# baoe/AlignGraph

Hardware: AMD Instinct MI355X
Metric: aligned reads/sec through graph build+extend (higher is better)
Workload: dtype u32

## Files before the change

### aligngraph_amd/csrc/agx_walk.cpp

```cpp
#include "agx_host.h"

#include <algorithm>
#include <atomic>
#include <thread>
#include <chrono>
#include <cstdio>
#include <cstdlib>
#include <cstring>
#include <deque>
#include <memory>
#include <memory_resource>
#include <string>
#include <vector>
#include <unordered_map>
#if defined(__x86_64__)
#include <immintrin.h>
#endif

#if defined(AGX_WALK_PROF) && defined(__x86_64__)
#include <x86intrin.h>
static unsigned long long g_prof[12];
#define AGX_PT(i) do { _mm_lfence(); const unsigned long long t_ = __rdtsc(); g_prof[i] += t_ - tp_; tp_ = t_; } while (0)
#define AGX_PT_START _mm_lfence(); unsigned long long tp_ = __rdtsc()
#else
// ... 224 lines not shown
        copies = nullptr;
    }
    bool may_look(agx_u32 v) const { if (!spec) return true; const agx_u32 x = pos_of(v); if (x >= look_lo && x < look_hi) return true; invalid = true; gave_up_at = x; return false; }
    std::vector<agx_edge_ovf> ovf;
    Walker(const UnitView &v, const GraphView &g) : V(v), G(g) {
        if (g.meta_rw) { if (g.meta_rw != g.meta) throw Error{E_ARG, "meta_rw must be the meta array"}; m = g.meta_rw; }
        else {
            const size_t n = (size_t)g.n_ids + 64;
            owned = (agx_u8 *)malloc(n); if (!owned) throw Error{E_ARG, "out of host memory"};
            advise_huge(owned, n); memcpy(owned, g.meta, n); m = owned;
        }
        for (size_t i = 0; i < g.n_ovf; i++) if (g.ovf[i].src != AGX_NONE) ovf.push_back(g.ovf[i]);
        std::sort(ovf.begin(), ovf.end(), [](const agx_edge_ovf &a, const agx_edge_ovf &b) { return a.src != b.src ? a.src < b.src : a.dst < b.dst; });
        ovf.erase(std::unique(ovf.begin(), ovf.end(), [](const agx_edge_ovf &a, const agx_edge_ovf &b) { return a.src == b.src && a.dst == b.dst; }), ovf.end());
    }
    mutable unsigned long long n_fetched = 0;
    mutable std::unordered_map<agx_u32, agx_walknode> extra;
    mutable std::vector<agx_walknode> rows;
    mutable agx_u32 last_v = AGX_NONE, last_at = AGX_NONE;
    agx_u32 rank_of(agx_u32 v) const {
        if (v == last_v) return last_at;
        const unsigned long long w = G.sp_bits[v >> 6], bit = 1ull << (v & 63u);
        last_v = v;
        return last_at = (w & bit) ? G.sp_rank[v >> 6] + (agx_u32)__builtin_popcountll(w & (bit - 1)) : AGX_NONE;
    }
    agx_hop hop_of(agx_u32 v, agx_u32 x) const {
        const agx_u32 r = G.sp_hop ? rank_of(v) : AGX_NONE;
        if (r != AGX_NONE) return G.sp_hop[r];
        if (V.hop) return V.hop[x];
        agx_hop h{0, 0, 0};
        if (!V.segs || V.n_seg0 == 0 || V.cm_count(x) != 1) return h;
        agx_u32 lo = 0, hi = V.n_seg0;
        while (hi - lo > 1) { const agx_u32 mid = lo + (hi - lo) / 2; if (V.segs[mid].pos0 <= x) lo = mid; else hi = mid; }
        const agx_cmseg &g = V.segs[lo];
        const agx_u32 j = x - g.pos0;
        if (x < g.pos0 || j >= g.len || j >= g.hop_len0) return h;
        h.str_off = g.hop_str0 + j; h.len = g.hop_len0 - j; h.end_pos = g.hop_end;
        return h;
    }
    agx_walknode node(agx_u32 v) const {
        const agx_u32 at = rank_of(v);
        if (at != AGX_NONE) {
            if (G.sp_hop) { __builtin_prefetch(G.sp_hop + at); __builtin_prefetch(G.sp_hop + at + 8); }
            __builtin_prefetch(G.sp_node + at + 6);
            return G.sp_node[at];
        }
        const auto it = extra.find(v);
        if (it != extra.end()) return it->second;
        if (!G.fetch) throw Error{E_ARG, "walk graph without a record fetch hook"};
        agx_walknode r; G.fetch(G.fetch_ctx, v, 1, 1, 1, &r); n_fetched++;
        extra.emplace(v, r);
        return r;
    }
    void prefetch_skip_positions(agx_u32 cp, agx_u32 end) const {
        if (!G.fetch || cp + 1000 >= end) return;
        const agx_u32 n = (end - cp - 1) / 1000;
        rows.resize((size_t)n * 2);
        G.fetch(G.fetch_ctx, cp + 999, 1000, n, 2, rows.data());
        for (agx_u32 i = 0; i < n; i++) { extra.emplace(cp + 999 + i * 1000, rows[2 * (size_t)i]); extra.emplace(cp + 1000 + i * 1000, rows[2 * (size_t)i + 1]); }
    }
    agx_u32 pos_of(agx_u32 v) const { return v < G.n_pos ? v : G.side_xpos[v - G.n_pos]; }
    void side_range(agx_u32 x, agx_u32 &lo, agx_u32 &hi) const {
        AGX_WCHK(*this, x, "side_range");
        if (!(m[x] & AGX_WM_SIDE)) { lo = hi = G.n_pos; return; }
        const agx_u32 *b = G.side_xpos, *e = G.side_xpos + (G.n_ids - G.n_pos);
        const agx_u32 *l = std::lower_bound(b, e, x), *h = l;
        while (h < e && *h == x) h++;
        lo = G.n_pos + (agx_u32)(l - b); hi = G.n_pos + (agx_u32)(h - b);
    }
    int live_successors(agx_u32 v, agx_u32 &target) const {
        AGX_WCHK(*this, v, "live_successors");
        if (m[v] & AGX_WM_CONT) { if (spec && v >= G.n_pos && !may_look(v + 1)) return 2; if (visited(v + 1)) return 0; target = v + 1; return 1; }
        int n = 0;
        const agx_walknode rec = node(v);
        const agx_u32 *s = rec.next;
        for (agx_u32 e = 0; e < AGX_MAXE && s[e] != AGX_NONE; e++) { if (!may_look(s[e])) return 2; if (!visited(s[e])) { target = s[e]; if (++n > 1) return n; } }
        if (!ovf.empty()) {
            auto it = std::lower_bound(ovf.begin(), ovf.end(), v, [](const agx_edge_ovf &a, agx_u32 key) { return a.src < key; });
            for (; it != ovf.end() && it->src == v; ++it) {
                bool inl = false; for (agx_u32 e = 0; e < AGX_MAXE; e++) inl |= s[e] == it->dst;
                if (!inl) { if (!may_look(it->dst)) return 2; if (!visited(it->dst)) { target = it->dst; if (++n > 1) return n; } }
            }
        }
        return n;
    }
    void kmer_string(agx_u32 v, std::string &out) const {
        agx_sref r = node(v).sref;
        if (V.slot_row) r.slot = V.slot_row[r.slot];
        const agx_u32 first = r.qlen & 0xFFFFu, len = (r.qlen >> 16) & 0x7FFFu; const bool rev = (r.qlen >> 31) != 0;
        out.clear();
        if (!V.bases) {
            if (!V.codes2) throw Error{E_ARG, "no read bases for the k-mer strings"};
            const agx_u8 *row = V.codes2 + (size_t)r.slot * (V.stride / 4);
            const unsigned long long base = (unsigned long long)r.slot * V.stride;
            for (agx_u32 i = 0; i < len; i++) {
                const agx_u32 j = rev ? first - i : first + i;
                char c = "ACGT"[(row[j >> 2] >> (2u * (j & 3u))) & 3u];
                if (c == 'A' && V.n_other) {
                    const unsigned long long *e = V.other_idx + V.n_other, *at = std::lower_bound(V.other_idx, e, base + j);
                    if (at != e && *at == base + j) c = (char)V.other_byte[at - V.other_idx];
                }
                out.push_back(!rev ? c : c == 'A' ? 'T' : c == 'C' ? 'G' : c == 'G' ? 'C' : c == 'T' ? 'A' : c);
            }
            return;
        }
        const char *p = V.row_off ? V.bases + V.row_off[r.slot] : V.bases + (size_t)(G.row_slot ? G.row_slot[r.slot] : r.slot) * V.stride;
        for (agx_u32 i = 0; i < len; i++) {
            if (!rev) out.push_back(p[first + i]);
            else { const char c = p[first - i]; out.push_back(c == 'A' ? 'T' : c == 'C' ? 'G' : c == 'G' ? 'C' : c == 'T' ? 'A' : c); }
        }
    }
    next_zero_fn next_zero = pick_next_zero();
    agx_u32 next_live(agx_u32 from, agx_u32 n) const { return from < n ? next_zero(m, from, n) : n; }
};

struct WalkState {
    agx_u32 cp = 0;
    agx_u32 seqID = 0, sIDBak = AGX_NONE, sOffBak = AGX_NONE, eIDBak = AGX_NONE, eOffBak = AGX_NONE;
    agx_u32 pos_bak = 0;
    bool same_scan(const WalkState &o) const { return cp == o.cp && sIDBak == o.sIDBak && sOffBak == o.sOffBak && eIDBak == o.eIDBak && eOffBak == o.eOffBak && pos_bak == o.pos_bak; }
};
typedef std::vector<std::pair<agx_u32, agx_u32>> MarkLog;

struct WalkRun {
    Walker &W; Arena *arena;
    WalkState st;
    std::vector<Rec> &written; PreFormat *pre;
    std::vector<PreJob> jobs;
    bool keep = true;
    MarkLog *log = nullptr; agx_u32 log_main = 0, log_side = 0;
    const std::atomic<bool> *cancel = nullptr;
    unsigned long long n_walks = 0, n_hops = 0, n_runs = 0, n_general = 0, run_nodes = 0;
    WalkRun(Walker &w, Arena *a, std::vector<Rec> &out, PreFormat *p) : W(w), arena(a), written(out), pre(p) {}
    void note_marks(agx_u32 a, agx_u32 b) {
        if (a < W.G.n_pos) { if (b >= log_main) log->push_back({a < log_main ? log_main : a, b}); }
        else if (b >= log_side) log->push_back({a < log_side ? log_side : a, b});
    }
    void go(agx_u32 stop) {
        const GraphView &G = W.G; const UnitView &V = W.V;
        agx_u32 &seqID = st.seqID, &sIDBak = st.sIDBak, &sOffBak = st.sOffBak, &eIDBak = st.eIDBak, &eOffBak = st.eOffBak, &pos_bak = st.pos_bak;
        std::string kmer; agx_u32 klen = 0, klast = 0;
        agx_hop hcur{0, 0, 0};
        std::vector<Seg> segs;
        agx_u8 *const m = W.m;
        auto done = [m, this](agx_u32 v) { AGX_WCHK(W, v, "done"); (void)this; return (m[v] & AGX_WM_VISITED) != 0; };
        const mark_fn mark = pick_mark();
        AGX_PT_START;
        const run_end_fn run_end = pick_run_end();
        const agx_u32 n_side = G.n_ids - G.n_pos;
        if (stop > G.n_pos) stop = G.n_pos;
        agx_u32 sc = (agx_u32)(std::lower_bound(G.side_xpos, G.side_xpos + n_side, st.cp) - G.side_xpos);
        agx_u32 side_live = G.n_pos + sc, main_live = st.cp;
        agx_u32 cp = st.cp;
        for (; cp < stop;) {
            if (W.invalid || (cancel && cancel->load(std::memory_order_relaxed))) break;
            while (sc < n_side && G.side_xpos[sc] < cp) sc++;
            agx_u32 sh = sc; while (sh < n_side && G.side_xpos[sh] == cp) sh++;
            const agx_u32 s_lo = G.n_pos + sc, s_hi = G.n_pos + sh;
            for (agx_u32 vi = 0, start = cp; vi <= s_hi - s_lo; vi++, start = s_lo + vi - 1) {
                if (done(start)) continue;
                AGX_PT(8);
                Rec C(arena); C.sID = 0; C.sOff = cp; C.extended = 0;
                segs.clear(); n_walks++;
                agx_u32 cur = start;
                AGX_PT(0);
                agx_u32 cpp = cp; int mode = 1;
                agx_u32 last = cur;
                while ((mode == 1 && !done(cur)) || mode == 0) {
                    if (mode == 0) {
                        AGX_PT(7); const agx_hop h = hcur;
                        segs.push_back(Seg{V.chain_str + h.str_off, h.len}); C.extended = 1; n_hops++;
                        pos_bak = h.end_pos; cpp = h.end_pos;
                        if (!W.may_look(cpp)) { mode = -2; break; }
                        agx_u32 live = 0, item = 0;
                        if (!done(cpp)) { live++; item = cpp; }
                        agx_u32 h_lo, h_hi; W.side_range(cpp, h_lo, h_hi);
                        for (agx_u32 v = h_lo; v < h_hi; v++) if (!done(v)) { live++; item = v; }
                        agx_u32 tgt = 0; int ns = 0;
                        if (live == 1) ns = W.live_successors(item, tgt);
                        if (ns == 1) { cur = tgt; pos_bak = W.pos_of(tgt); cpp = pos_bak; mode = done(cur) ? -2 : 1; }
                        else mode = -2;
                        AGX_PT(1);
                    } else {
                        agx_u8 seen = 0;
                        AGX_WCHK(W, cur, "run start");
                        const agx_u32 j = run_end(m, cur, seen);
                        const agx_u32 xj = j < G.n_ids ? W.pos_of(j) : 0xFFFFFFFFu;
                        if (W.spec && (xj < W.look_lo || xj >= W.look_hi || (j >= G.n_pos && j + 1 < G.n_ids && W.pos_of(j + 1) >= W.look_hi))) { W.invalid = true; W.gave_up_at = xj; mode = -2; break; }
                        AGX_PT(2);
                        AGX_WCHK(W, j, "run end"); if (j + 1 < G.n_ids && (j + 1 < G.n_pos) == (j < G.n_pos)) AGX_WCHK(W, j + 1, "behind the run");
                        segs.push_back(Seg{G.str + cur, (size_t)j - cur + 1}); n_runs++; run_nodes += j - cur + 1; if (!(m[j] & AGX_WM_CONT)) n_general++;
                        if (seen & AGX_WM_CONTIG) C.extended = 1;
                        if (W.copies) W.before_mark(j);
                        mark(m, cur, j);
                        if (log && j >= log_main) note_marks(cur, j);
                        if (j > cur) pos_bak = xj;
                        cur = j; last = j; cpp = xj;
                        AGX_PT(3);
                        agx_u32 tgt = 0;
                        const int ns = (m[cur] & AGX_WM_CONT) ? 0 : W.live_successors(cur, tgt);
                        if (ns == 1) { cur = tgt; pos_bak = W.pos_of(tgt); cpp = pos_bak; }
                        else if ((hcur = W.hop_of(j, xj)).len) mode = 0;
                        else mode = -1;
                        AGX_PT(4);
                    }
                }
                C.eID = 0; C.eOff = mode == 1 ? pos_bak : cpp;
                if (mode == 1 || mode == -1) {
                    { const agx_u32 o = W.node(cur).off0; C.eID0 = o == AGX_NONE ? AGX_NONE : 0; C.eOff0 = o; }
                    klen = (W.node(last).sref.qlen >> 16) & 0x7FFFu; klast = last;
                    C.eOff = C.eOff + klen - 1; C.eOff0 = C.eOff0 + klen - 1;
                } else { C.eID0 = AGX_NONE; C.eOff0 = AGX_NONE; klen = 0; }
                AGX_PT(5);
                if (!contains(sIDBak, sOffBak, eIDBak, eOffBak, C.sID, C.sOff, C.eID, C.eOff)) {
                    { const agx_u32 o = W.node(start).off0; C.sID0 = o == AGX_NONE ? AGX_NONE : 0; C.sOff0 = o; }
                    if (klen > 1) {
                        W.kmer_string(klast, kmer);
                        char *t = (char *)arena->allocate(kmer.size() - 1, 1); memcpy(t, kmer.data() + 1, kmer.size() - 1);
                        segs.push_back(Seg{t, kmer.size() - 1});
                    }
                    C.nuc.segs.reserve(segs.size());
                    for (const Seg &g : segs) C.nuc.add(g.p, g.n);
                    sIDBak = C.sID; sOffBak = C.sOff; eIDBak = C.eID; eOffBak = C.eOff;
                    if (eOffBak - sOffBak > 100000) W.prefetch_skip_positions(cp, eOffBak < G.n_pos ? eOffBak : G.n_pos);
                    if (keep) {
                        PreJob j; const agx_u32 f[10] = {seqID, (agx_u32)C.extended, C.sID, C.sOff, C.eID, C.eOff, C.sID0, C.sOff0, C.eID0, C.eOff0};
                        memcpy(j.f, f, sizeof f); j.segs = C.nuc.segs.data(); j.n_segs = C.nuc.segs.size(); j.total = C.nuc.len;
                        if (pre) pre->add(j); else jobs.push_back(j);
                        written.push_back(std::move(C));
                    }
                    seqID++;
                }
                AGX_PT(6);
            }
            AGX_PT(9);
            if (eOffBak - sOffBak > 100000 && eIDBak == 0 && cp + 1000 < eOffBak) cp += 1000;
            else {
                auto stale = [m](agx_u32 v) { return (m[v] & AGX_WM_VISITED) != 0; };
                if (main_live <= cp || (main_live < G.n_pos && stale(main_live))) main_live = W.next_live(main_live > cp + 1 ? main_live : cp + 1, G.n_pos);
                const agx_u32 m = main_live;
                if (side_live < s_hi || (side_live < G.n_ids && stale(side_live))) side_live = W.next_live(side_live > s_hi ? side_live : s_hi, G.n_ids);
                const agx_u32 sd = side_live;
                const agx_u32 sp = sd < G.n_ids ? G.side_xpos[sd - G.n_pos] : G.n_pos;
                cp = m < sp ? m : sp;
                if (cp >= W.scan_hi) { W.invalid = true; W.gave_up_at = cp; }
            }
            AGX_PT(10);
    }
        st.cp = cp;
    }
};

inline void walk_report(const WalkRun &r) {
#if defined(AGX_WALK_PROF) && defined(__x86_64__)
    if (getenv("AGX_WALK_TIMING")) {
        fprintf(stderr, "[agx walk] Mcycles: start %.1f, hop %.1f, run scan %.1f, mark %.1f, successors %.1f, end %.1f, contain+write %.1f, between %.1f, position scan %.1f (+ %.1f after the last variant, %.1f next position)\n",
                g_prof[0] / 1e6, g_prof[1] / 1e6, g_prof[2] / 1e6, g_prof[3] / 1e6, g_prof[4] / 1e6, g_prof[5] / 1e6, g_prof[6] / 1e6, g_prof[7] / 1e6, g_prof[8] / 1e6, g_prof[9] / 1e6, g_prof[10] / 1e6);
        memset(g_prof, 0, sizeof g_prof);
    }
#endif
    if (getenv("AGX_WALK_TIMING")) fprintf(stderr, "[agx walk] walks %llu, contig hops %llu, runs %llu (%llu nodes), general evaluations %llu\n", r.n_walks, r.n_hops, r.n_runs, r.run_nodes, r.n_general);
}

void walk(Walker &W, OutBuf &pre_out, std::vector<Rec> &written, Arena *arena, Assistant *assistant, WalkPaths *paths) {
    if (W.G.wait_landed) W.G.wait_landed(W.G.land_ctx, W.G.n_pos, W.G.n_ids);
    if (W.G.wait_str) W.G.wait_str(W.G.land_ctx);
    pre_out.reserve((size_t)W.G.n_ids + W.G.n_ids / 32 + 4096);
    PreFormat pre(pre_out, assistant, (size_t)W.G.n_pos / 256 + 65536);
    pre.paths = paths; pre.graph = &W.G;
    WalkRun run(W, arena, written, &pre);
    run.go(W.G.n_pos);
    pre.finish();
    walk_report(run);
}

inline std::atomic<double> &walker_speed() { static std::atomic<double> v{700000.0}; return v; }
inline void clip_marks(const MarkLog &log, agx_u32 main_lo, agx_u32 main_hi, agx_u32 n_pos, agx_u32 side_lo, agx_u32 side_hi, MarkLog &out) {
    out.clear();
    for (const auto &r : log) {
        agx_u32 a = r.first, b = r.second;
        if (b < n_pos) { if (a < main_lo) a = main_lo; if (b >= main_hi) { if (main_hi == 0) continue; b = main_hi - 1; } }
        else { if (a < side_lo) a = side_lo; if (b >= side_hi) { if (side_hi == 0) continue; b = side_hi - 1; } }
        if (a <= b) out.push_back({a, b});
    }
    std::sort(out.begin(), out.end());
    size_t k = 0;
    for (size_t i = 0; i < out.size(); i++) {
        if (k && out[i].first <= out[k - 1].second + 1) { if (out[i].second > out[k - 1].second) out[k - 1].second = out[i].second; }
        else out[k++] = out[i];
    }
    out.resize(k);
}

struct SpecWalker {
    agx_u32 c = 0, c_next = 0, w0 = 0, side_c = 0, side_next = 0, warm_lo = 0, warm_hi = 0xFFFFFFFFu, look_hi = 0, win_lo = 0, win_hi = 0, side_win_hi = 0, copy_hi = 0, side_copy_lo = 0, side_copy_hi = 0;
    Scratch bytes;
    GraphView G; std::unique_ptr<Walker> W; std::unique_ptr<WalkRun> R; std::vector<Rec> recs;
    MarkLog log; size_t n_warm = 0;
    WalkState at_c;
    bool ok = false; std::string error;
    double t_run = 0, t_copy = 0, t_warm = 0, t_done = 0;
};

bool walk_split(Walker &WA, const UnitView &V, const GraphView &G, OutBuf &pre_out, std::vector<Rec> &written, Arena *arena, Arena *const *more_arenas, Assistant *assistant, WalkPaths *paths) {
    const agx_u32 min_ref = getenv("AGX_WALK_SPLIT_MIN") ? (agx_u32)strtoul(getenv("AGX_WALK_SPLIT_MIN"), nullptr, 10) : 4000000u;
    agx_u32 warm = 400000u;
    if (const char *e = getenv("AGX_WALK_SPLIT_WARMUP")) warm = (agx_u32)strtoul(e, nullptr, 10);
    else if (V.segs) {
        agx_u32 reach = 0;
        for (agx_u32 i = 0; i < V.n_seg0; i++) { const agx_cmseg &g = V.segs[i]; if (g.hop_len0 && g.hop_end > g.pos0 && g.hop_end - g.pos0 > reach) reach = g.hop_end - g.pos0; }
        const unsigned long long w = 3ull * reach + 20000ull;
        warm = (agx_u32)(w < 100000ull ? 100000ull : w > 400000ull ? 400000ull : w);
    }
    const agx_u32 n_ref = V.n_ref < G.n_pos ? V.n_ref : G.n_pos;
    if (!assistant || n_ref < min_ref || n_ref < 16 || getenv("AGX_WALK_NO_SPLIT")) return false;
    int K = walkers_for(n_ref);
    if (K > 1 + assistant->helpers()) K = 1 + assistant->helpers();
    const agx_u32 slack = 64;
    if (K > (int)(n_ref / (8 * slack))) K = (int)(n_ref / (8 * slack));
    if (K < 2) return false;
    const agx_u32 lead = n_ref / (unsigned)K > 4 * warm ? 2 * warm : 0;
    std::vector<agx_u32> cuts((size_t)K + 1, n_ref); cuts[0] = 0;
    for (int i = 1; i < K; i++) cuts[(size_t)i] = lead + (agx_u32)((unsigned long long)(n_ref - lead) * (unsigned)i / (unsigned)K);
    const bool streamed = G.wait_landed != nullptr && G.land_ms > 0;
    if (!getenv("AGX_WALK_EVEN_CUTS")) {
        const double v = walker_speed().load(), D = streamed ? G.land_ms : 0.0, copy_ms = 0.15 + 3.2 * ((double)n_ref / K) / 12e6, warm_ms = 2.0 * (double)warm / v, floor_len = std::max(1024.0, (double)n_ref / (16.0 * K));
        std::vector<double> len((size_t)K, (double)n_ref / K), ready((size_t)K, 0.0), at((size_t)K + 1, 0.0);
        for (int round = 0; round < 6; round++) {
            for (int i = 0; i < K; i++) at[(size_t)i + 1] = at[(size_t)i] + len[(size_t)i];
            double sum = ready[0] = D;
            for (int i = 1; i < K; i++) { const double hi = i + 2 >= K ? (double)G.n_pos : std::max(at[(size_t)i + 2], at[(size_t)i + 1] + (double)warm); sum += ready[(size_t)i] = D * std::min(1.0, hi / (double)G.n_pos) + copy_ms + warm_ms; }
            const double T = ((double)n_ref / v + sum) / K;
            double total = 0;
            for (int i = 0; i < K; i++) total += len[(size_t)i] = std::max(v * (T - ready[(size_t)i]), floor_len);
            for (int i = 0; i < K; i++) len[(size_t)i] *= (double)n_ref / total;
        }
        double acc = 0;
        for (int i = 1; i < K; i++) { acc += len[(size_t)i - 1]; const agx_u32 lo = cuts[(size_t)i - 1] + 8 * slack, hi = n_ref - (agx_u32)(K - i) * 8 * slack; const agx_u32 c = (agx_u32)acc; cuts[(size_t)i] = c < lo ? lo : c > hi ? hi : c; }
    }
    auto cut_at = [&](int i) { return i >= K ? n_ref : i <= 0 ? 0u : cuts[(size_t)i]; };
    const agx_u32 n_side = G.n_ids - G.n_pos;
    auto side_of = [&](agx_u32 x) { return G.n_pos + (agx_u32)(std::lower_bound(G.side_xpos, G.side_xpos + n_side, x) - G.side_xpos); };
    const agx_u32 side_ref = side_of(n_ref);
    pre_out.reserve((size_t)G.n_ids + G.n_ids / 32 + 4096);
    const bool timing = getenv("AGX_WALK_TIMING") != nullptr;
    auto clock = [] { return std::chrono::duration<double, std::milli>(std::chrono::steady_clock::now().time_since_epoch()).count(); };

    const double t_enter = clock();
    std::atomic<bool> cancel{false};
    std::atomic<int> copied{0};
    const agx_u8 *const pristine = WA.m;
    std::vector<SpecWalker> B((size_t)K - 1);
    for (int i = 1; i < K; i++) {
        SpecWalker &b = B[(size_t)i - 1];
        b.c = cut_at(i); b.c_next = cut_at(i + 1);
        b.side_c = side_of(b.c); b.side_next = side_of(b.c_next);
        int ahead = i + 2; while (ahead < K && cut_at(ahead) < b.c_next + warm) ahead++;
        const bool open_end = ahead >= K;
        const agx_u32 back = 2 * warm + slack < b.c - cut_at(i - 1) ? 2 * warm + slack : b.c - cut_at(i - 1);
        b.win_lo = b.c - back; b.win_hi = open_end ? n_ref : cut_at(ahead); b.side_win_hi = open_end ? side_ref : side_of(b.win_hi);
        b.copy_hi = open_end ? G.n_pos : b.win_hi; b.side_copy_lo = side_of(b.win_lo); b.side_copy_hi = open_end ? G.n_ids : b.side_win_hi;
        b.warm_lo = b.win_lo ? b.win_lo + slack : 0; b.warm_hi = open_end ? 0xFFFFFFFFu : b.win_hi - slack; b.look_hi = open_end ? n_ref : b.win_hi - slack;
        b.w0 = b.c > warm ? b.c - warm : 0; if (b.w0 < b.warm_lo) b.w0 = b.warm_lo;
        b.bytes.take((size_t)G.n_ids + 64);
        b.G = G; b.G.meta = (const agx_u8 *)b.bytes.p; b.G.meta_rw = (agx_u8 *)b.bytes.p;
        b.W.reset(new Walker(V, b.G));
        b.recs.reserve((size_t)G.n_pos / 2048 + 1024);
        b.R.reset(new WalkRun(*b.W, more_arenas[i - 1], b.recs, nullptr));
    }
    struct Join { Assistant *a; int n; std::atomic<bool> &c; std::vector<bool> joined; void now(int i) { if (!joined[(size_t)i]) { a->wait(i); joined[(size_t)i] = true; } } ~Join() { c.store(true); for (int i = 0; i < n; i++) now(i); } } join{assistant, K - 1, cancel, std::vector<bool>((size_t)K - 1, false)};
    for (int i = 1; i < K; i++) {
        SpecWalker *bp = &B[(size_t)i - 1];
        assistant->run([bp, &cancel, &copied, pristine, &G, n_ref, side_ref] {
            SpecWalker &b = *bp; Walker &W = *b.W; WalkRun &R = *b.R;
            auto clk = [] { return std::chrono::duration<double, std::milli>(std::chrono::steady_clock::now().time_since_epoch()).count(); };
            b.t_run = clk();
            struct Copied { std::atomic<int> &n; bool done = false; void now() { if (!done) { done = true; n.fetch_add(1, std::memory_order_release); } } ~Copied() { now(); } } copied_mark{copied};
            try {
                if (const char *pz = getenv("AGX_WALK_POISON")) { const long v = strtol(pz, nullptr, 0); memset(W.m, v > 1 ? (int)(v & 0xFF) : 0xA5, (size_t)G.n_ids + 64); }
                if (G.wait_landed) G.wait_landed(G.land_ctx, b.copy_hi, b.side_copy_hi);
                memcpy(W.m + b.win_lo, pristine + b.win_lo, (size_t)b.copy_hi - b.win_lo);
                memcpy(W.m + b.side_copy_lo, pristine + b.side_copy_lo, (size_t)b.side_copy_hi - b.side_copy_lo + (b.side_copy_hi == G.n_ids ? 64 : 0));
                if (b.copy_hi < G.n_pos) W.m[b.copy_hi] = AGX_WM_VISITED;
                if (b.side_copy_hi < G.n_ids) W.m[b.side_copy_hi] = AGX_WM_VISITED;
                copied_mark.now(); b.t_copy = clk();
                W.spec = true; W.look_lo = b.warm_lo; W.look_hi = b.warm_hi; W.scan_hi = b.warm_hi;
#ifdef AGX_WALK_CHECK
                W.chk_lo = b.win_lo; W.chk_hi = b.copy_hi; W.chk_slo = b.side_copy_lo; W.chk_shi = b.side_copy_hi;
#endif
                R.cancel = &cancel; R.st.cp = b.w0; R.keep = false; R.log = &b.log; R.log_main = 0; R.log_side = G.n_pos;
                R.go(b.c);
                b.at_c = R.st; b.n_warm = b.log.size(); b.t_warm = clk();
                for (const auto &r : b.log) for (agx_u32 v = r.first; v <= r.second; v++) if (v < G.n_pos ? v >= n_ref : v >= side_ref) W.m[v] &= (agx_u8)~AGX_WM_VISITED;
                R.keep = true; R.st.seqID = 0;
                if (b.c_next < n_ref) { R.log_main = b.c_next; R.log_side = b.side_next; } else R.log = nullptr;
                W.look_lo = b.c; W.look_hi = b.look_hi;
                if (const char *e = getenv("AGX_WALK_SPLIT_LOOK")) { const unsigned long long hi = (unsigned long long)b.c + strtoull(e, nullptr, 10); if (hi < W.look_hi) W.look_hi = (agx_u32)hi; }
                if (!W.invalid && !cancel.load()) R.go(b.c_next);
                b.ok = !W.invalid && !cancel.load() && R.st.cp >= b.c_next; b.t_done = clk();
            } catch (const Error &e) { b.error = e.msg; } catch (const std::exception &e) { b.error = e.what(); }
        }, i - 1);
    }
    WA.copies = &copied; WA.copies_want = K - 1; WA.guard_main = B[0].win_lo; WA.guard_side = B[0].side_copy_lo;
    struct Unguard { Walker &w; ~Unguard() { w.copies = nullptr; } } unguard{WA};
    if (G.wait_landed) G.wait_landed(G.land_ctx, G.n_pos, G.n_ids);

    const double tw0 = clock();
    MarkLog log_a;
    WalkRun A(WA, arena, written, nullptr);
    A.log = &log_a; A.log_main = B[0].c; A.log_side = B[0].side_c;
    A.go(B[0].c);
    A.log = nullptr;
    const size_t a_first = A.jobs.size();
    const double tw1 = clock();
    const MarkLog *truth = &log_a; WalkState at = A.st; int stood = 0; MarkLog ma, mb;
    for (int i = 1; i < K; i++) {
        SpecWalker &b = B[(size_t)i - 1];
        join.now(i - 1);
        bool same = b.ok && b.error.empty() && at.same_scan(b.at_c);
        if (same) {
            MarkLog warm_marks(b.log.begin(), b.log.begin() + (long)b.n_warm);
            clip_marks(*truth, b.c, n_ref, G.n_pos, b.side_c, side_ref, ma); clip_marks(warm_marks, b.c, n_ref, G.n_pos, b.side_c, side_ref, mb);
            same = ma == mb;
        }
        if (timing) {
            if (same) fprintf(stderr, "[agx walk] walker %d of %d, [%u, %u) after a warm-up from %u: its stretch stands (began at %.2f ms, window %.2f ms, warm-up %.2f ms, stretch %.2f ms)\n", i + 1, K, b.c, b.c_next, b.w0, b.t_run - t_enter, b.t_copy - b.t_run, b.t_warm - b.t_copy, b.t_done - b.t_warm);
            else if (!b.error.empty()) fprintf(stderr, "[agx walk] walker %d of %d failed (%s): walked on by the first walker from %u\n", i + 1, K, b.error.c_str(), b.c);
            else if (b.W->invalid) fprintf(stderr, "[agx walk] walker %d of %d gave up (a walk led to position %u, outside [%u, %u)): walked on by the first walker from %u\n", i + 1, K, b.W->gave_up_at, b.W->look_lo, b.W->look_hi, b.c);
            else fprintf(stderr, "[agx walk] walker %d of %d, [%u, %u) after a warm-up from %u: states differ at the meeting point (scan at %u / %u, last record %u..%u / %u..%u, %zu / %zu mark ranges): walked on by the first walker\n",
                         i + 1, K, b.c, b.c_next, b.w0, at.cp, b.at_c.cp, at.sOffBak, at.eOffBak, b.at_c.sOffBak, b.at_c.eOffBak, ma.size(), mb.size());
        }
        if (!same) break;
        const agx_u32 shift = at.seqID;
        for (PreJob &j : b.R->jobs) j.f[0] += shift;
        at = b.R->st; at.seqID = shift + b.R->st.seqID;
        truth = &b.log; stood = i;
    }
    cancel.store(true);
    for (int i = stood; i < K - 1; i++) join.now(i);
    WA.copies = nullptr;
    {
        double pos = 0, ms = 0;
        for (int i = 1; i <= stood; i++) { const SpecWalker &b = B[(size_t)i - 1]; if (b.t_done > b.t_warm) { pos += (double)(b.c_next - b.c); ms += b.t_done - b.t_warm; } }
        if (ms > 0.05 && pos > 1e5) { const double seen = pos / ms, old = walker_speed().load(); walker_speed().store(0.7 * old + 0.3 * std::min(std::max(seen, 1e5), 5e6)); }
    }
    const double tw2 = clock();
    if (!(stood == K - 1 && WA.next_live(n_ref, G.n_pos) >= G.n_pos && WA.next_live(side_ref, G.n_ids) >= G.n_ids)) {
        auto merge = [&WA](const agx_u8 *src, agx_u32 lo, agx_u32 hi) {
            agx_u32 v = lo;
            for (; v < hi && (v & 7u); v++) WA.m[v] |= (agx_u8)(src[v] & AGX_WM_VISITED);
            for (; v + 8 <= hi; v += 8) { uint64_t x, y; memcpy(&x, WA.m + v, 8); memcpy(&y, src + v, 8); x |= y & 0x8080808080808080ull; memcpy(WA.m + v, &x, 8); }
            for (; v < hi; v++) WA.m[v] |= (agx_u8)(src[v] & AGX_WM_VISITED);
        };
        auto merge_of = [&](int i) {
            const SpecWalker &b = B[(size_t)i - 1]; const agx_u8 *src = b.W->m;
            if (i < stood) { merge(src, b.c, b.c_next); merge(src, b.side_c, b.side_next); } else { merge(src, b.c, b.win_hi); merge(src, b.side_c, b.side_win_hi); }
        };
        struct Wait { Assistant *a; int n; ~Wait() { for (int i = 0; i < n; i++) a->wait(i); } } wait{assistant, stood > 1 ? stood - 1 : 0};
        for (int i = 1; i < stood; i++) assistant->run([&merge_of, i] { merge_of(i); }, i - 1);
        if (stood) merge_of(stood);
    }
    for (int i = 1; i <= stood; i++) {
        SpecWalker &b = B[(size_t)i - 1];
        for (Rec &r : b.recs) written.push_back(std::move(r));
        WA.n_fetched += b.W->n_fetched;
        A.n_walks += b.R->n_walks; A.n_hops += b.R->n_hops; A.n_runs += b.R->n_runs; A.n_general += b.R->n_general; A.run_nodes += b.R->run_nodes;
    }
    if (stood) A.st = at;
    const double tw3 = clock();
    A.go(G.n_pos);
    const double tw4 = clock();
    std::vector<PreJob> all;
    all.insert(all.end(), A.jobs.begin(), A.jobs.begin() + (long)a_first);
    for (int i = 1; i <= stood; i++) all.insert(all.end(), B[(size_t)i - 1].R->jobs.begin(), B[(size_t)i - 1].R->jobs.end());
    all.insert(all.end(), A.jobs.begin() + (long)a_first, A.jobs.end());
    if (paths) for (const PreJob &j : all) note_paths(j, G, *paths);
    std::vector<size_t> place(all.size() + 1, 0);
    auto header_len = [](const PreJob &j) { size_t n = 1 + 9 * 2 + 2; for (int i = 0; i < 10; i++) { agx_u32 v = j.f[i]; do { n++; v /= 10u; } while (v); } return n; };
    for (size_t i = 0; i < all.size(); i++) place[i + 1] = place[i] + header_len(all[i]) + all[i].total + (all[i].total + 59) / 60;
    const size_t total = place[all.size()];
    if (G.wait_str) G.wait_str(G.land_ctx);
    pre_out.n = 0; char *base = pre_out.grow(total);
    auto format = [&](size_t lo, size_t hi) {
        for (size_t i = lo; i < hi; i++) {
            const PreJob &j = all[i];
            char *h = base + place[i]; *h++ = '>';
            for (int f = 0; f < 10; f++) { h = put_u32(h, j.f[f]); if (f < 9) { *h++ = ','; *h++ = ' '; } }
            *h++ = ' '; *h++ = '\n';
            LineWriter lw(h); for (size_t g = 0; g < j.n_segs; g++) lw.put(j.segs[g].p, j.segs[g].n); lw.end();
        }
    };
    {
        const int shares = total > (1u << 16) ? K : 1;
        std::vector<size_t> cut((size_t)shares + 1, all.size()); cut[0] = 0;
        for (int t = 1; t < shares; t++) { size_t m = cut[(size_t)t - 1]; while (m < all.size() && place[m] < total / (unsigned)shares * (unsigned)t) m++; cut[(size_t)t] = m; }
        struct Wait { Assistant *a; int n; ~Wait() { for (int i = 0; i < n; i++) a->wait(i); } } wait{assistant, shares - 1};
        for (int t = 0; t + 1 < shares; t++) { const size_t lo = cut[(size_t)t], hi = cut[(size_t)t + 1]; assistant->run([&format, lo, hi] { format(lo, hi); }, t); }
        format(cut[(size_t)shares - 1], all.size());
    }
    if (timing) fprintf(stderr, "[agx walk] first walker began at %.2f ms; %u appended positions behind the reference%s\n", tw0 - t_enter, G.n_pos - n_ref, streamed ? " (streamed download: stretches cut by when their windows land)" : "");
    if (timing && streamed) { fprintf(stderr, "[agx walk] cuts (%.1f ms of download left at the start, %.0f positions per ms):", G.land_ms, walker_speed().load()); for (int i = 1; i < K; i++) fprintf(stderr, " %u", cuts[(size_t)i]); fprintf(stderr, "\n"); }
    if (timing) fprintf(stderr, "[agx walk] %d walkers, %d stretches stood: first stretch %.1f ms, waited %.1f ms for the others, merge %.1f ms, rest %.1f ms, formatting %.1f ms\n", K, stood, tw1 - tw0, tw2 - tw1, tw3 - tw2, tw4 - tw3, clock() - tw4);
    walk_report(A);
    return true;
}

}

namespace {

void join(std::vector<Rec> &c) {
    const int n = (int)c.size();
    for (int cp = 0; cp < n; cp++) if (c[cp].extended == 1)
        for (int q = cp + 1; q < n; q++) {
            if (contains(c[cp].sID, c[cp].sOff, c[cp].eID, c[cp].eOff, c[q].sID, c[q].sOff, c[q].eID, c[q].eOff)) c[q].extended = 2;
            else if (c[cp].eID != c[q].sID || c[cp].eOff < c[q].sOff) break;
        }
    for (int cp = n - 1; cp >= 0; cp--) if (c[cp].extended == 1)
        for (int q = cp - 1; q >= 0; q--) {
            if (contains(c[cp].sID, c[cp].sOff, c[cp].eID, c[cp].eOff, c[q].sID, c[q].sOff, c[q].eID, c[q].eOff)) c[q].extended = 2;
            else if (c[q].eID != c[cp].sID || c[q].eOff < c[cp].sOff) break;
        }
    for (int cp = 0; cp < n; cp++) {
        while (c[cp].extended == 1) {
            int cand = -1, ncand = 0;
            for (int q = cp + 1; q < n; q++) if (c[q].extended != 2) { if (c[cp].eOff >= c[q].sOff) { cand = q; ncand++; } else break; }
            if (ncand != 1) break;
            Rec &d = c[cand]; d.extended = 2;
            const size_t from = (size_t)(int)(c[cp].eOff - d.sOff + 1);
            if (from < d.nuc.len) c[cp].nuc.add_from(d.nuc, from);
            c[cp].eID = d.eID; c[cp].eOff = d.eOff; c[cp].eID0 = d.eID0; c[cp].eOff0 = d.eOff0;
        }
    }
}

inline int overlaps(agx_u32 x1, agx_u32 y1, agx_u32 x2, agx_u32 y2) {
    return (x1 <= x2 && x2 <= y1 && y1 <= y2 && (int)y1 - (int)x2 > 0) || (x2 <= x1 && x1 <= y2 && y2 <= y1 && (int)y2 - (int)x1 > 0) ||
           (x1 <= x2 && x2 <= y2 && y2 <= y1 && (int)y2 - (int)x2 > 0) || (x2 <= x1 && x1 <= y1 && y1 <= y2 && (int)y1 - (int)x1 > 0);
}

void scaffold(const UnitView &V, const GraphView &G, std::vector<Rec> &c, OutBuf &out, Arena *arena, Assistant *assistant) {
    std::vector<Bases> sc; sc.reserve(c.size());
    const agx_u32 n = (agx_u32)c.size();
    std::vector<agx_u32> s_off(n); agx_u32 longest = 0; bool ordered = true;
    for (agx_u32 i = 0; i < n; i++) {
        s_off[i] = c[i].sOff;
        if (i && s_off[i] < s_off[i - 1]) ordered = false;
        if (c[i].eOff < c[i].sOff) longest = 0xFFFFFFFFu; else if (c[i].eOff - c[i].sOff > longest) longest = c[i].eOff - c[i].sOff;
    }
    for (agx_u32 cp = 0; cp < n; cp++) {
        if (!(c[cp].sID != AGX_NONE && c[cp].extended == 1)) continue;
        sc.push_back(std::move(c[cp].nuc)); c[cp].nuc = Bases(arena); c[cp].sID = AGX_NONE;
        bool cont = true;
        while (c[cp].sID0 == c[cp].eID0 && cont) {
            cont = false;
            agx_u32 q = cp + 1;
            if (ordered && longest != 0xFFFFFFFFu && c[cp].sOff0 > longest) {
                const agx_u32 from = (agx_u32)(std::lower_bound(s_off.begin(), s_off.end(), c[cp].sOff0 - longest) - s_off.begin());
                if (from > q) q = from;
            }
            for (; q < n; q++) {
                if (ordered && c[q].sOff > c[cp].eOff0) break;
                if (!(c[cp].eID0 == c[q].sID && c[q].sID == c[q].eID && overlaps(c[cp].sOff0, c[cp].eOff0, c[q].sOff, c[q].eOff) && c[q].extended == 1)) continue;
                if (c[q].sOff > c[cp].eOff) {
                    const agx_u32 gap = c[q].sOff - c[cp].eOff - 1; agx_u32 covered = 0;
                    for (agx_u32 i = 0; i < gap; i++) { const agx_u32 x = c[cp].eOff + i + 1; if ((G.meta[x] & AGX_WM_ANY) || V.has_cm(x)) covered++; }
                    if (gap == 0 || (double)(int)covered / gap >= 0.5) sc.back().add(V.ref + c[cp].eOff + 1, gap);
                    else continue;
                }
                sc.back().add_from(c[q].nuc, 0); c[q].sID = AGX_NONE; cp = q; cont = true;
                break;
            }
        }
    }
    const double t_dec = std::chrono::duration<double, std::milli>(std::chrono::steady_clock::now().time_since_epoch()).count();
    std::vector<size_t> at(sc.size() + 1, 0);
    auto header = [](char *hdr, size_t i) { char *h = hdr; *h++ = '>'; char t[24]; int n = 0; do { t[n++] = (char)('0' + i % 10); i /= 10; } while (i); while (n) *h++ = t[--n]; *h++ = '\n'; return (size_t)(h - hdr); };
    for (size_t i = 0; i < sc.size(); i++) { char hdr[32]; at[i + 1] = at[i] + header(hdr, i) + sc[i].len + (sc[i].len + 59) / 60; }
    const size_t total = at[sc.size()];
    out.n = 0; char *base = out.grow(total);
    auto format = [&](size_t lo, size_t hi) {
        for (size_t i = lo; i < hi; i++) {
            char hdr[32]; const size_t hl = header(hdr, i);
            char *w = base + at[i]; memcpy(w, hdr, hl);
            LineWriter lw(w + hl); lw.put(sc[i]); lw.end();
        }
    };
    const int shares = assistant && total > (1u << 16) ? std::min(8, 1 + assistant->helpers()) : 1;
    if (shares > 1) {
        std::vector<size_t> cut((size_t)shares + 1, sc.size()); cut[0] = 0;
        for (int t = 1; t < shares; t++) { size_t m = cut[(size_t)t - 1]; while (m < sc.size() && at[m] < total / (unsigned)shares * (unsigned)t) m++; cut[(size_t)t] = m; }
        struct Wait { Assistant *a; int n; ~Wait() { for (int i = 0; i < n; i++) a->wait(i); } } wait{assistant, shares - 1};
        for (int t = 0; t + 1 < shares; t++) { const size_t lo = cut[(size_t)t], hi = cut[(size_t)t + 1]; assistant->run([&format, lo, hi] { format(lo, hi); }, t); }
        format(cut[(size_t)shares - 1], sc.size());
    } else format(0, sc.size());
    if (getenv("AGX_WALK_TIMING")) fprintf(stderr, "[agx walk] scaffold: output %.1f ms of it (%zu scaffolds, %zu bytes)\n", std::chrono::duration<double, std::milli>(std::chrono::steady_clock::now().time_since_epoch()).count() - t_dec, sc.size(), total);
}

}

void build_chains(Threads &T) {
    const size_t n = T.cm.size(), n_pos = T.ref.size();
    T.chain_off.assign(1, 0); T.chain_end_pos.clear(); T.chain_str.clear();
    T.chain_str.reserve(n);
    T.hop.assign(n_pos, agx_hop{0, 0, 0});
    std::vector<agx_u8> state(n, 0);
    auto index_of = [&](agx_u32 off, agx_u32 item) -> size_t {
        if (off >= n_pos || T.cm_start[off] + item >= T.cm_start[off + 1]) throw Error{E_ARG, "conti-mer link to a missing entry"};
        return (size_t)T.cm_start[off] + item;
    };
    for (size_t i = 0; i < n; i++) if (T.cm[i].next_off != AGX_NONE) state[index_of(T.cm[i].next_off, T.cm[i].next_item)] = 1;
    std::vector<agx_u32> pending;
    size_t visited = 0;
    T.segs.clear(); T.n_seg0 = 0;
    for (size_t x = 0; x < n_pos; x++) for (size_t h = T.cm_start[x]; h < T.cm_start[x + 1]; h++) {
        if (state[h]) continue;
        pending.clear();
        size_t c = h; agx_u32 pos = (agx_u32)x;
        const size_t seg_first = T.segs.size(), str_base = T.chain_str.size();
        for (agx_u32 i = 0;; i++) {
            if (state[c] == 2) throw Error{E_ARG, "conti-mer chains are not simple lists"};
            state[c] = 2; visited++;
            T.chain_str.push_back(T.cm[c].nuc);
            const ContiMer &m = T.cm[c];
            {
                const agx_u32 rank = (agx_u32)(c - T.cm_start[pos]);
                agx_cmseg *g = T.segs.size() > seg_first ? &T.segs.back() : nullptr;
                const bool joins = g && pos == g->pos0 + g->len && rank == g->rank && m.cid == g->cid && (g->len == 1 || m.coff == g->coff0 + g->len * g->dcoff);
                if (joins) { if (g->len == 1) g->dcoff = m.coff - g->coff0; g->len++; }
                else T.segs.push_back(agx_cmseg{pos, 1u, m.cid, m.coff, 0u, rank, (agx_u32)(str_base + i + 1), i, 0u, 0u});
            }
            if (m.next_off == AGX_NONE) break;
            if (T.cm_start[pos + 1] - T.cm_start[pos] == 1) { T.hop[pos].str_off = (agx_u32)T.chain_str.size(); pending.push_back(pos); }
            c = index_of(m.next_off, m.next_item); pos = m.next_off;
        }
        if (T.chain_str.size() >= 0xFFFFFFFFull) throw Error{E_ARG, "conti-mer chains exceed 2^32 bases"};
        for (agx_u32 p : pending) { T.hop[p].len = (agx_u32)(T.chain_str.size() - T.hop[p].str_off); T.hop[p].end_pos = pos; }
        {   const agx_u32 last = (agx_u32)(T.chain_str.size() - str_base - 1);
            for (size_t g = seg_first; g < T.segs.size(); g++) { T.segs[g].hop_len0 = last - T.segs[g].hop_len0; T.segs[g].hop_end = pos; } }
        T.chain_end_pos.push_back(pos); T.chain_off.push_back(T.chain_str.size());
    }
    if (visited != n) throw Error{E_ARG, "conti-mer cycle"};
    std::stable_sort(T.segs.begin(), T.segs.end(), [](const agx_cmseg &a, const agx_cmseg &b) { return (a.rank != 0) != (b.rank != 0) ? a.rank == 0 : (a.rank == 0 && a.pos0 < b.pos0); });
    agx_u32 e = 0;
    for (agx_cmseg &g : T.segs) { g.elem0 = e; e += g.len; if (g.rank == 0) T.n_seg0++; }
    if (e != n) throw Error{E_ARG, "conti-mer runs do not cover the conti-mers"};
    T.n_cm = n; T.cm_cnt.resize(n_pos);
    for (size_t x = 0; x < n_pos; x++) { const agx_u32 c = T.cm_start[x + 1] - T.cm_start[x]; if (c > 255) throw Error{E_UNSUPPORTED, "more than 255 conti-mers at one position"}; T.cm_cnt[x] = (agx_u8)c; }
}

void walk_join_scaffold(const UnitView &V, const GraphView &G, UnitOutput &out, Assistant *assistant) {
    if (!V.hop && !G.sp_hop && !V.segs) throw Error{E_ARG, "conti-mer chains were not built"};
    const bool timing = getenv("AGX_WALK_TIMING") != nullptr;
    auto now = [] { return std::chrono::duration<double, std::milli>(std::chrono::steady_clock::now().time_since_epoch()).count(); };
    const double ts = now();
    Walker W(V, G);
    std::pmr::monotonic_buffer_resource arena((size_t)8 << 20);
    std::vector<std::unique_ptr<std::pmr::monotonic_buffer_resource>> others;
    Arena *more_arenas[GraphView::MAX_WALKERS - 1];
    for (int i = 0; i < GraphView::MAX_WALKERS - 1; i++) { others.emplace_back(new std::pmr::monotonic_buffer_resource((size_t)1 << 20)); more_arenas[i] = others.back().get(); }
    std::vector<Rec> recs; recs.reserve((size_t)G.n_pos / 1024 + 1024);
    double t0 = now();
    WalkPaths *paths = out.keep_paths ? &out.paths : nullptr;
    if (!walk_split(W, V, G, out.pre_extended, recs, &arena, more_arenas, assistant, paths)) walk(W, out.pre_extended, recs, &arena, assistant, paths);
    double t1 = now();
    join(recs);
    double t2 = now();
    scaffold(V, G, recs, out.extended, &arena, assistant);
    double t3 = now();
    out.n_fetched = W.n_fetched;
    if (timing) fprintf(stderr, "[agx walk] set-up %.2f ms, walk %.2f ms, join %.2f ms, scaffold %.1f ms, %zu records, %u special ids of %u, %llu records fetched\n", t0 - ts, t1 - t0, t2 - t1, t3 - t2, recs.size(), G.n_special, G.n_ids, W.n_fetched);
}

}
```

Before: 1.343 billion.

## Overlap pre-extended output formatting with join and scaffold decisions

Moves the pre-extended FASTA formatting out of walk_split into a PreTail object. Helper threads format the output in dynamically claimed pieces while the unit's thread runs join and the scaffold decisions, and the unit's thread joins in and waits for the helpers before writing the scaffold output. This is meant to take the formatting off the critical path after the last walk stretch. It also replaces the fixed per-walker shares with work-stealing pieces and adds timing instrumentation, at the cost of helper threads being busy when scaffold later wants them.

```diff
diff --git a/aligngraph_amd/csrc/agx_walk.cpp b/aligngraph_amd/csrc/agx_walk.cpp
--- a/aligngraph_amd/csrc/agx_walk.cpp
+++ b/aligngraph_amd/csrc/agx_walk.cpp
@@ -550,7 +550,73 @@
     double t_run = 0, t_copy = 0, t_warm = 0, t_done = 0;
 };
 
-bool walk_split(Walker &WA, const UnitView &V, const GraphView &G, OutBuf &pre_out, std::vector<Rec> &written, Arena *arena, Arena *const *more_arenas, Assistant *assistant, WalkPaths *paths) {
+struct PreTail {
+    std::vector<PreJob> all;
+    std::vector<size_t> place, cut;
+    std::atomic<size_t> next{0};
+    char *base = nullptr; size_t total = 0;
+    const GraphView *G = nullptr; Assistant *assistant = nullptr; int running = 0;
+    bool timing = false; double t_walked = 0, t_started = 0;
+    struct Lap { double begin = 0, bases = 0, end = 0; size_t pieces = 0, bytes = 0; } lap[GraphView::MAX_WALKERS + 1];
+    static double clock() { return std::chrono::duration<double, std::milli>(std::chrono::steady_clock::now().time_since_epoch()).count(); }
+    void format(size_t lo, size_t hi) const {
+        for (size_t i = lo; i < hi; i++) {
+            const PreJob &j = all[i];
+            char *h = base + place[i]; *h++ = '>';
+            for (int f = 0; f < 10; f++) { h = put_u32(h, j.f[f]); if (f < 9) { *h++ = ','; *h++ = ' '; } }
+            *h++ = ' '; *h++ = '\n';
+            LineWriter lw(h); for (size_t g = 0; g < j.n_segs; g++) lw.put(j.segs[g].p, j.segs[g].n); lw.end();
+        }
+    }
+    void work(int who) {
+        Lap &l = lap[who];
+        if (timing) l.begin = clock();
+        if (next.load(std::memory_order_relaxed) + 1 >= cut.size()) { l.bases = l.end = l.begin; return; }
+        if (G->wait_str) G->wait_str(G->land_ctx);
+        if (timing) l.bases = clock();
+        for (;;) {
+            const size_t p = next.fetch_add(1, std::memory_order_relaxed);
+            if (p + 1 >= cut.size()) break;
+            format(cut[p], cut[p + 1]); l.pieces++; l.bytes += place[cut[p + 1]] - place[cut[p]];
+        }
+        if (timing) l.end = clock();
+    }
+    void start(const GraphView &g, OutBuf &out, Assistant *a, int helpers, double walked) {
+        G = &g; timing = getenv("AGX_WALK_TIMING") != nullptr; t_walked = walked;
+        place.assign(all.size() + 1, 0);
+        auto header_len = [](const PreJob &j) { size_t n = 1 + 9 * 2 + 2; for (int i = 0; i < 10; i++) { agx_u32 v = j.f[i]; do { n++; v /= 10u; } while (v); } return n; };
+        for (size_t i = 0; i < all.size(); i++) place[i + 1] = place[i] + header_len(all[i]) + all[i].total + (all[i].total + 59) / 60;
+        total = place[all.size()];
+        out.n = 0; base = out.grow(total);
+        if (helpers > GraphView::MAX_WALKERS) helpers = GraphView::MAX_WALKERS;
+        const size_t small = (size_t)1 << 16; size_t piece = total <= small ? total + 1 : std::max((size_t)1 << 18, total / (4 * ((size_t)helpers + 1)));
+        if (const char *e = getenv("AGX_WALK_TAIL_PIECE")) { if (total > small) piece = std::max((size_t)1, (size_t)strtoull(e, nullptr, 10)); }
+        cut.assign(1, 0);
+        for (size_t i = 0; i < all.size();) { size_t m = i + 1; while (m < all.size() && place[m] - place[i] < piece) m++; cut.push_back(m); i = m; }
+        if (total > small && a) { assistant = a; for (int t = 0; t < helpers; t++) { a->run([this, t] { work(t); }, t); running = t + 1; } }
+        if (timing) t_started = clock();
+    }
+    void join_helpers() { while (running > 0) assistant->wait(--running); }
+    void finish() {
+        if (!G) return;
+        const double t0 = timing ? clock() : 0;
+        work(GraphView::MAX_WALKERS); join_helpers();
+        if (!timing) return;
+        const double t1 = clock(); const Lap &me = lap[GraphView::MAX_WALKERS];
+        double b0 = 1e30, b1 = 0, w0 = 1e30, w1 = 0, c0 = 1e30, c1 = 0, end = t_started; size_t n = 0;
+        for (int t = 0; t < GraphView::MAX_WALKERS; t++) { const Lap &l = lap[t]; if (l.begin == 0) continue; n++;
+            b0 = std::min(b0, l.begin - t_started); b1 = std::max(b1, l.begin - t_started); w0 = std::min(w0, l.bases - l.begin); w1 = std::max(w1, l.bases - l.begin);
+            c0 = std::min(c0, l.end - l.bases); c1 = std::max(c1, l.end - l.bases); end = std::max(end, l.end); }
+        if (!n) b0 = w0 = c0 = 0;
+        fprintf(stderr, "[agx walk] pre-extended formatting beside join and scaffold: places and hand-over %.2f ms behind the last stretch; %zu helpers began %.2f .. %.2f ms later, waited %.2f .. %.2f ms for the bases, "
+                "copied for %.2f .. %.2f ms, the last one done %.2f ms behind the last stretch; %zu bytes in %zu pieces\n", t_started - t_walked, n, b0, b1, w0, w1, c0, c1, end - t_walked, total, cut.size() - 1);
+        fprintf(stderr, "[agx walk] the unit's thread: join and the scaffold's decisions until %.2f ms behind the last stretch, then %zu pieces (%zu bytes, %.2f ms of it waiting for the bases) and %.2f ms waiting for the helpers: formatting done at %.2f ms\n",
+                t0 - t_walked, me.pieces, me.bytes, me.bases - me.begin, t1 - std::max(me.end, t0), t1 - t_walked);
+    }
+    ~PreTail() { if (running > 0) { next.store(cut.size(), std::memory_order_relaxed); join_helpers(); } }
+};
+
+bool walk_split(Walker &WA, const UnitView &V, const GraphView &G, OutBuf &pre_out, std::vector<Rec> &written, Arena *arena, Arena *const *more_arenas, Assistant *assistant, WalkPaths *paths, PreTail &tail) {
     const agx_u32 min_ref = getenv("AGX_WALK_SPLIT_MIN") ? (agx_u32)strtoul(getenv("AGX_WALK_SPLIT_MIN"), nullptr, 10) : 4000000u;
     agx_u32 warm = 400000u;
     if (const char *e = getenv("AGX_WALK_SPLIT_WARMUP")) warm = (agx_u32)strtoul(e, nullptr, 10);
@@ -718,37 +784,15 @@
     const double tw3 = clock();
     A.go(G.n_pos);
     const double tw4 = clock();
-    std::vector<PreJob> all;
+    std::vector<PreJob> &all = tail.all;
     all.insert(all.end(), A.jobs.begin(), A.jobs.begin() + (long)a_first);
     for (int i = 1; i <= stood; i++) all.insert(all.end(), B[(size_t)i - 1].R->jobs.begin(), B[(size_t)i - 1].R->jobs.end());
     all.insert(all.end(), A.jobs.begin() + (long)a_first, A.jobs.end());
+    tail.start(G, pre_out, assistant, K - 1, tw4);
     if (paths) for (const PreJob &j : all) note_paths(j, G, *paths);
-    std::vector<size_t> place(all.size() + 1, 0);
-    auto header_len = [](const PreJob &j) { size_t n = 1 + 9 * 2 + 2; for (int i = 0; i < 10; i++) { agx_u32 v = j.f[i]; do { n++; v /= 10u; } while (v); } return n; };
-    for (size_t i = 0; i < all.size(); i++) place[i + 1] = place[i] + header_len(all[i]) + all[i].total + (all[i].total + 59) / 60;
-    const size_t total = place[all.size()];
-    if (G.wait_str) G.wait_str(G.land_ctx);
-    pre_out.n = 0; char *base = pre_out.grow(total);
-    auto format = [&](size_t lo, size_t hi) {
-        for (size_t i = lo; i < hi; i++) {
-            const PreJob &j = all[i];
-            char *h = base + place[i]; *h++ = '>';
-            for (int f = 0; f < 10; f++) { h = put_u32(h, j.f[f]); if (f < 9) { *h++ = ','; *h++ = ' '; } }
-            *h++ = ' '; *h++ = '\n';
-            LineWriter lw(h); for (size_t g = 0; g < j.n_segs; g++) lw.put(j.segs[g].p, j.segs[g].n); lw.end();
-        }
-    };
-    {
-        const int shares = total > (1u << 16) ? K : 1;
-        std::vector<size_t> cut((size_t)shares + 1, all.size()); cut[0] = 0;
-        for (int t = 1; t < shares; t++) { size_t m = cut[(size_t)t - 1]; while (m < all.size() && place[m] < total / (unsigned)shares * (unsigned)t) m++; cut[(size_t)t] = m; }
-        struct Wait { Assistant *a; int n; ~Wait() { for (int i = 0; i < n; i++) a->wait(i); } } wait{assistant, shares - 1};
-        for (int t = 0; t + 1 < shares; t++) { const size_t lo = cut[(size_t)t], hi = cut[(size_t)t + 1]; assistant->run([&format, lo, hi] { format(lo, hi); }, t); }
-        format(cut[(size_t)shares - 1], all.size());
-    }
     if (timing) fprintf(stderr, "[agx walk] first walker began at %.2f ms; %u appended positions behind the reference%s\n", tw0 - t_enter, G.n_pos - n_ref, streamed ? " (streamed download: stretches cut by when their windows land)" : "");
     if (timing && streamed) { fprintf(stderr, "[agx walk] cuts (%.1f ms of download left at the start, %.0f positions per ms):", G.land_ms, walker_speed().load()); for (int i = 1; i < K; i++) fprintf(stderr, " %u", cuts[(size_t)i]); fprintf(stderr, "\n"); }
-    if (timing) fprintf(stderr, "[agx walk] %d walkers, %d stretches stood: first stretch %.1f ms, waited %.1f ms for the others, merge %.1f ms, rest %.1f ms, formatting %.1f ms\n", K, stood, tw1 - tw0, tw2 - tw1, tw3 - tw2, tw4 - tw3, clock() - tw4);
+    if (timing) fprintf(stderr, "[agx walk] %d walkers, %d stretches stood: first stretch %.1f ms, waited %.1f ms for the others, merge %.1f ms, rest %.1f ms, formatting handed over in %.2f ms\n", K, stood, tw1 - tw0, tw2 - tw1, tw3 - tw2, tw4 - tw3, clock() - tw4);
     walk_report(A);
     return true;
 }
@@ -759,16 +803,22 @@
 
 void join(std::vector<Rec> &c) {
     const int n = (int)c.size();
+    const bool timing = getenv("AGX_WALK_TIMING") != nullptr;
+    auto clock = [] { return std::chrono::duration<double, std::milli>(std::chrono::steady_clock::now().time_since_epoch()).count(); };
+    const double t0 = timing ? clock() : 0;
     for (int cp = 0; cp < n; cp++) if (c[cp].extended == 1)
         for (int q = cp + 1; q < n; q++) {
             if (contains(c[cp].sID, c[cp].sOff, c[cp].eID, c[cp].eOff, c[q].sID, c[q].sOff, c[q].eID, c[q].eOff)) c[q].extended = 2;
             else if (c[cp].eID != c[q].sID || c[cp].eOff < c[q].sOff) break;
         }
+    const double t1 = timing ? clock() : 0;
     for (int cp = n - 1; cp >= 0; cp--) if (c[cp].extended == 1)
         for (int q = cp - 1; q >= 0; q--) {
             if (contains(c[cp].sID, c[cp].sOff, c[cp].eID, c[cp].eOff, c[q].sID, c[q].sOff, c[q].eID, c[q].eOff)) c[q].extended = 2;
             else if (c[q].eID != c[cp].sID || c[q].eOff < c[cp].sOff) break;
         }
+    const double t2 = timing ? clock() : 0;
+    size_t appended = 0;
     for (int cp = 0; cp < n; cp++) {
         while (c[cp].extended == 1) {
             int cand = -1, ncand = 0;
@@ -777,9 +827,10 @@
             Rec &d = c[cand]; d.extended = 2;
             const size_t from = (size_t)(int)(c[cp].eOff - d.sOff + 1);
             if (from < d.nuc.len) c[cp].nuc.add_from(d.nuc, from);
-            c[cp].eID = d.eID; c[cp].eOff = d.eOff; c[cp].eID0 = d.eID0; c[cp].eOff0 = d.eOff0;
-        }
-    }
+            c[cp].eID = d.eID; c[cp].eOff = d.eOff; c[cp].eID0 = d.eID0; c[cp].eOff0 = d.eOff0; appended++;
+        }
+    }
+    if (timing) fprintf(stderr, "[agx walk] join: contained behind %.2f ms, contained in front %.2f ms, appends %.2f ms (%zu of %d records appended)\n", t1 - t0, t2 - t1, clock() - t2, appended, n);
 }
 
 inline int overlaps(agx_u32 x1, agx_u32 y1, agx_u32 x2, agx_u32 y2) {
@@ -787,7 +838,8 @@
            (x1 <= x2 && x2 <= y2 && y2 <= y1 && (int)y2 - (int)x2 > 0) || (x2 <= x1 && x1 <= y1 && y1 <= y2 && (int)y1 - (int)x1 > 0);
 }
 
-void scaffold(const UnitView &V, const GraphView &G, std::vector<Rec> &c, OutBuf &out, Arena *arena, Assistant *assistant) {
+void scaffold(const UnitView &V, const GraphView &G, std::vector<Rec> &c, OutBuf &out, Arena *arena, Assistant *assistant, PreTail &tail) {
+    const double t_in = std::chrono::duration<double, std::milli>(std::chrono::steady_clock::now().time_since_epoch()).count();
     std::vector<Bases> sc; sc.reserve(c.size());
     const agx_u32 n = (agx_u32)c.size();
     std::vector<agx_u32> s_off(n); agx_u32 longest = 0; bool ordered = true;
@@ -822,6 +874,8 @@
         }
     }
     const double t_dec = std::chrono::duration<double, std::milli>(std::chrono::steady_clock::now().time_since_epoch()).count();
+    tail.finish();
+    const double t_pre = std::chrono::duration<double, std::milli>(std::chrono::steady_clock::now().time_since_epoch()).count();
     std::vector<size_t> at(sc.size() + 1, 0);
     auto header = [](char *hdr, size_t i) { char *h = hdr; *h++ = '>'; char t[24]; int n = 0; do { t[n++] = (char)('0' + i % 10); i /= 10; } while (i); while (n) *h++ = t[--n]; *h++ = '\n'; return (size_t)(h - hdr); };
     for (size_t i = 0; i < sc.size(); i++) { char hdr[32]; at[i + 1] = at[i] + header(hdr, i) + sc[i].len + (sc[i].len + 59) / 60; }
@@ -842,7 +896,7 @@
         for (int t = 0; t + 1 < shares; t++) { const size_t lo = cut[(size_t)t], hi = cut[(size_t)t + 1]; assistant->run([&format, lo, hi] { format(lo, hi); }, t); }
         format(cut[(size_t)shares - 1], sc.size());
     } else format(0, sc.size());
-    if (getenv("AGX_WALK_TIMING")) fprintf(stderr, "[agx walk] scaffold: output %.1f ms of it (%zu scaffolds, %zu bytes)\n", std::chrono::duration<double, std::milli>(std::chrono::steady_clock::now().time_since_epoch()).count() - t_dec, sc.size(), total);
+    if (getenv("AGX_WALK_TIMING")) fprintf(stderr, "[agx walk] scaffold: decisions %.2f ms, %.2f ms for the rest of the pre-extended output, output %.2f ms on %d shares (%zu scaffolds, %zu bytes)\n", t_dec - t_in, t_pre - t_dec, std::chrono::duration<double, std::milli>(std::chrono::steady_clock::now().time_since_epoch()).count() - t_pre, shares, sc.size(), total);
 }
 
 }
@@ -910,13 +964,15 @@
     std::vector<Rec> recs; recs.reserve((size_t)G.n_pos / 1024 + 1024);
     double t0 = now();
     WalkPaths *paths = out.keep_paths ? &out.paths : nullptr;
-    if (!walk_split(W, V, G, out.pre_extended, recs, &arena, more_arenas, assistant, paths)) walk(W, out.pre_extended, recs, &arena, assistant, paths);
+    PreTail tail;
+    if (!walk_split(W, V, G, out.pre_extended, recs, &arena, more_arenas, assistant, paths, tail)) walk(W, out.pre_extended, recs, &arena, assistant, paths);
     double t1 = now();
     join(recs);
     double t2 = now();
-    scaffold(V, G, recs, out.extended, &arena, assistant);
+    scaffold(V, G, recs, out.extended, &arena, assistant, tail);
     double t3 = now();
     out.n_fetched = W.n_fetched;
+    if (timing && tail.t_walked > 0) fprintf(stderr, "[agx walk] tail behind the last stretch: %.2f ms on the unit's thread (pre-extended formatting, join, scaffold)\n", t3 - tail.t_walked);
     if (timing) fprintf(stderr, "[agx walk] set-up %.2f ms, walk %.2f ms, join %.2f ms, scaffold %.1f ms, %zu records, %u special ids of %u, %llu records fetched\n", t0 - ts, t1 - t0, t2 - t1, t3 - t2, recs.size(), G.n_special, G.n_ids, W.n_fetched);
 }
 
```

Result: no change. 1.329 billion (median of 2 runs) (-1.0%).
